# epam/ai-dial-rag

Hardware: AMD Instinct MI355X
Metric: retrieval_qps_10Mx384 (higher is better)
Workload: dtype f32 (int8 MFMA filter with exact integer dot products and a rigorous error margin, every candidate the margin cannot exclude re-scored in f64 with the reference formula)

## Files before the change

ai-dial-rag_amd/csrc/vec_index.hip:

```cpp
#include <algorithm>
#include <cmath>
#include <cstdarg>
#include <cstdio>
#include <cstdlib>
#include <cstring>
#include <mutex>
#include <new>
#include <type_traits>
#include <vector>

#include "common.h"
#include "vec_kernels.h"
#include "vec_kernels_f16.h"
#include "vec_kernels_q16.h"
#include "vec_kernels_h16.h"
#include "vec_kernels_sieve.h"
#include "vec_kernels_i8.h"
#include "vec_kernels_exact.h"

namespace mir {

static thread_local char g_err[512] = "";

void set_error(const char *fmt, ...) {
// ... 835 lines not shown
            sa.chunk_ids = ix->d_chunk; sa.doc_ids = ix->d_doc; sa.row_offset = ix->row_offset;
            sa.out_doc = o_doc; sa.out_chunk = o_chunk; sa.out_row = o_row; sa.out_dist = o_dist; sa.out_count = o_count;
            sa.out_flags = o_flags; sa.nflag = sb.nflag; sa.flagged = sb.flagged; sa.stats = ix->d_stats; sa.qt = sb.qt;
            rc = sieve(0, (uint32_t)kSampleWgs * pl.sample_tpw, kSampleWgs, nullptr, nullptr, nullptr, true);
            if (rc != MIR_OK) return rc;
            if (use_i8) {
                SieveSampleArgs ta;
                ta.part = reinterpret_cast<const float *>(sb.part_sample); ta.nwg = kSampleWgs; ta.qpw = qpw; ta.k = k; ta.nq = nq;
                ta.q0 = q0; ta.d = d; ta.metric = metric; ta.docs = ix->d_orig; ta.doc_sq = ix->d_docsq;
                ta.q = dq; ta.q_sq = sb.q_sq; ta.q_norm = sb.q_norm; ta.gthr = reinterpret_cast<unsigned long long *>(gt);
                sieve_sample_threshold_kernel<<<dim3(nq), dim3(256), 0, stream>>>(ta);
            } else {
                sample_threshold_kernel<<<dim3(nq), dim3(256), 0, stream>>>(reinterpret_cast<const float *>(sb.part_sample), kSampleWgs, qpw,
                                                                            k, nq, reinterpret_cast<unsigned long long *>(gt));
            }
            MIR_HIP(hipGetLastError());
            rc = begin_profile();
            if (rc != MIR_OK) return rc;
            for (int phase = pl.tiles_first ? 0 : 1; phase < 2 && rc == MIR_OK; ++phase) {
                const size_t region = use_i8 ? (size_t)kI8Region : (size_t)kSieveRegion;
                uint64_t *cand = sb.sv_cand + (size_t)phase * nwg * region;
                float *cv = sb.sv_candv + (size_t)phase * nwg * region;
                uint32_t *cc = sb.sv_ccount + (size_t)phase * nwg * (use_i8 ? 8 : 1);
                rc = phase == 0 ? sieve(0, pl.tiles_first, nwg, cand, cv, cc, false)
                                : sieve(pl.tiles_first, ix->n_tiles - pl.tiles_first, nwg, cand, cv, cc, false);
                if (rc != MIR_OK) break;
                if (phase == 1 && ev0) {
                    MIR_HIP(hipEventRecord(ev1, stream));
                    std::lock_guard<std::mutex> lk(ix->mu);
                    ix->prof_events.emplace_back(ev0, ev1);
                    ev1 = nullptr;
                }
                ca.cand = cand; ca.candv = cv; ca.ccount = cc;
                if (use_i8) sieve_scatter_i8_kernel<<<dim3(nwg * 8), dim3(256), 0, stream>>>(ca);
                else sieve_scatter_kernel<<<dim3(nwg * kSieveScatterSplit), dim3(256), 0, stream>>>(ca);
                sa.mode = phase;
                MIR_HIP(hipFuncSetAttribute(reinterpret_cast<const void *>(sieve_select_kernel), hipFuncAttributeMaxDynamicSharedMemorySize,
                                            (int)sieve_select_lds_bytes()));
                sieve_select_kernel<<<dim3(nq), dim3(kSieveSelectThreads), sieve_select_lds_bytes(), stream>>>(sa);
                MIR_HIP(hipGetLastError());
            }
            if (rc != MIR_OK) return rc;
            continue;
        }
        rc = begin_profile();
        if (rc != MIR_OK) return rc;
        if (qpw == 32) {
            rc = with_kind(metric, [&](auto kind) { return launch_scan<kind()>(ix, qs, nq, klist, nwg, pg, stream); });
        } else if (ix->native16) {
            const uint4 *qs16 = sb.qsplit + (size_t)g * (kQ16Queries / 16) * (ix->ksteps / 2) * 64;
            const float *qsc = sb.qscale + (size_t)g * qpw;
            rc = with_kind(metric, [&](auto kind) { return launch_scan_h16<kind()>(ix, qs16, qsc, nq, klist, nwg, pg, sb.gthr + (size_t)g * 128, stream); });
        } else if (ix->layout16) {
            const double *qn = sb.q_norm + (size_t)g * qpw;
            rc = with_kind(metric, [&](auto kind) { return launch_scan_q16<kind()>(ix, qs, qn, nq, klist, nwg, pg, stream); });
        } else {
            rc = with_kind(metric, [&](auto kind) { return launch_scan_f16<kind()>(ix, qs, nq, klist, nwg, pg, stream); });
        }
        if (ev1) {
            (void)hipEventRecord(ev1, stream);
            std::lock_guard<std::mutex> lk(ix->mu);
            ix->prof_events.emplace_back(ev0, ev1);
        }
        if (rc != MIR_OK) return rc;
    }
    if (pl.sieve) {
// ... 8 lines not shown
    fa.q = dq; fa.q_sq = sb.q_sq; fa.q_norm = sb.q_norm;
    fa.chunk_ids = ix->d_chunk; fa.doc_ids = ix->d_doc; fa.row_offset = ix->row_offset;
    fa.out_doc = o_doc; fa.out_chunk = o_chunk; fa.out_row = o_row; fa.out_dist = o_dist;
    fa.out_count = o_count; fa.out_flags = o_flags; fa.nflag = sb.nflag; fa.flagged = sb.flagged; fa.qt = sb.qt;
    finalize_kernel<<<dim3(b), dim3(256), 0, stream>>>(fa);
    MIR_HIP(hipGetLastError());
    exact_pass();
    MIR_HIP(hipGetLastError());
    return MIR_OK;
}

static int32_t plan(const mir_index *ix, int b, int k, SearchPlan *pl) {
    {
        const int64_t per_wg = (int64_t)b * std::min(k, kExactRound) * 16;
        const int64_t by_mem = std::max<int64_t>(64, ((int64_t)256 << 20) / std::max<int64_t>(per_wg, 1));
        pl->exact_grid = (int)std::max<int64_t>(1, std::min<int64_t>(std::min<int64_t>(ix->num_cus, by_mem), (ix->n + kXbRows - 1) / kXbRows));
    }
    pl->klist = std::min(k + (ix->native16 ? kH16ListMargin : kListMargin), kMaxList);
    auto exact_only = [&]() {
        pl->exact_only = true;
        pl->ngroups = 0;
        pl->qpw = 32;
        pl->nwg = 1;
        return MIR_OK;
    };
    if (ix->hi_only || ix->wide16 || (ix->native16 && sieve_sized(ix))) {
        if (k > kSieveMaxK) return exact_only();
        pl->sieve = true;
        pl->qpw = (ix->layout16 && b > kQ16Queries) ? kSieveMaxQueriesPerLaunch : kQ16Queries;
        pl->ngroups = (b + pl->qpw - 1) / pl->qpw;
        pl->nwg = (int)std::min<int64_t>(std::min(ix->num_cus, 1024), (int64_t)ix->n_tiles);
        pl->klist = std::min(k, kMaxList);
        const bool two = (int64_t)ix->n_tiles >= (int64_t)kSieveTwoLaunchTiles * pl->nwg;
        pl->tiles_first = two ? std::max<uint32_t>(ix->n_tiles / kSieveFirstDiv, std::min<uint32_t>(ix->n_tiles / 4, kSieveFirstMinTiles)) : 0;
        pl->tiles_first &= ~1u;
        pl->sample_tpw = std::max<uint32_t>(1, std::min<uint32_t>(kSampleTilesPerWg, ix->n_tiles / (4u * kSampleWgs)));
        return MIR_OK;
    }
    const bool wide64 = wide64_split(ix);
    const bool lists_fit = k + (ix->native16 ? kH16ListMargin : kListMargin) <= kMaxList;
    if (!lists_fit && ix->n > (int64_t)kMaxList) return exact_only();
    if (wide64 && f16_lds_bytes(pl->klist) <= 160 * 1024) {
        pl->qpw = kF16Queries;
        pl->ngroups = (b + pl->qpw - 1) / pl->qpw;
        const int64_t want16 = (int64_t)ix->n_tiles;
        pl->nwg = (int)std::max<int64_t>(1, std::min<int64_t>(std::min(ix->num_cus, 1024), want16));
        return MIR_OK;
    }
    if ((ix->layout16 || ix->native16) && pl->klist > kQ16MaxList) return exact_only();
    if (ix->layout16 || ix->native16) {
        pl->qpw = kQ16Queries;
        pl->ngroups = (b + pl->qpw - 1) / pl->qpw;
        pl->nwg = (int)std::max<int64_t>(1, std::min<int64_t>(std::min(ix->num_cus, 1024), (int64_t)ix->n_tiles));
        return MIR_OK;
    }
    pl->qpw = 32;
    pl->ngroups = (b + pl->qpw - 1) / pl->qpw;
    const int64_t want = (int64_t)ix->n_tiles;
    pl->nwg = (int)std::max<int64_t>(1, std::min<int64_t>(std::min(ix->num_cus, 1024), want));
    return MIR_OK;
}

}


struct ConcatItem {
    const void *src;
    int64_t dst_unit;
    int32_t n_units;
// ... 320 lines not shown
    std::vector<std::pair<hipEvent_t, hipEvent_t>> ev;
    {
        std::lock_guard<std::mutex> lk(idx->mu);
        ev.swap(idx->prof_events);
    }
    double ms = 0.0;
    for (auto &pr : ev) {
        float t = 0.f;
        hipError_t e = hipEventSynchronize(pr.second);
        if (e == hipSuccess) e = hipEventElapsedTime(&t, pr.first, pr.second);
        {
            std::lock_guard<std::mutex> lk(idx->mu);
            idx->prof_free.push_back(pr.first);
            idx->prof_free.push_back(pr.second);
        }
        if (e != hipSuccess) {
            set_error("profile read failed: %s", hipGetErrorString(e));
            return MIR_ERR_HIP;
        }
        ms += t;
    }
    std::lock_guard<std::mutex> lk(idx->mu);
    idx->prof_launches += (int64_t)ev.size();
    idx->prof_ms += ms;
    if (launches) *launches = idx->prof_launches;
    if (total_ms) *total_ms = idx->prof_ms;
    if (reset) {
        idx->prof_launches = 0;
        idx->prof_ms = 0.0;
    }
    return MIR_OK;
}

int32_t mir_index_scan_stats(mir_index *idx, int32_t reset, int64_t *out8) {
    MIR_REQUIRE(idx != nullptr && out8 != nullptr, "NULL argument");
    int32_t rc = use_device(idx->device, nullptr);
    if (rc != MIR_OK) return rc;
    MIR_HIP(hipDeviceSynchronize());
    MIR_HIP(hipMemcpy(out8, idx->d_stats, 64, hipMemcpyDeviceToHost));
    if (reset) MIR_HIP(hipMemset(idx->d_stats, 0, 64));
    out8[6] = idx->i8 ? 1 : 0;
    return MIR_OK;
}

int32_t mir_index_search_device(mir_index *idx, const double *queries_device, int32_t b, int32_t k,
                                int32_t metric, int32_t *out_doc, int64_t *out_chunk, int64_t *out_row,
                                double *out_dist, int32_t *out_count, int32_t *out_flags, void *stream_) {
    int32_t rc = check_search_args(idx, queries_device, b, k, metric, out_count);
    if (rc != MIR_OK) return rc;
    if (b == 0) return MIR_OK;
    hipStream_t stream = static_cast<hipStream_t>(stream_);
    rc = use_device(idx->device, nullptr);
    if (rc != MIR_OK) return rc;
    SearchPlan pl;
    rc = plan(idx, b, k, &pl);
    if (rc != MIR_OK) return rc;
    SearchBuffers sb;
    const size_t i8_rows = (idx->i8 && pl.sieve) ? (size_t)idx->n_stages * 64 : 0;
    const size_t need = carve(sb, nullptr, b, k, idx->d, std::max(idx->ksteps, idx->ks16), pl, false, i8_rows);
    Workspace *w = nullptr;
    rc = acquire_ws(idx, stream, need, &w);
    if (rc != MIR_OK) return rc;
    carve(sb, static_cast<char *>(w->buf), b, k, idx->d, std::max(idx->ksteps, idx->ks16), pl, false, i8_rows);
    rc = enqueue_search(idx, queries_device, b, k, metric, sb, pl, out_doc, out_chunk, out_row,
                        out_dist, out_count, out_flags, stream);
    release_ws(idx, w, stream, true);
    return rc;
}

int32_t mir_index_search(mir_index *idx, const double *queries_host, int32_t b, int32_t k, int32_t metric,
                         int32_t *out_doc, int64_t *out_chunk, int64_t *out_row, double *out_dist,
                         int32_t *out_count, int32_t *out_flags) {
    int32_t rc = check_search_args(idx, queries_host, b, k, metric, out_count);
    if (rc != MIR_OK) return rc;
// ... 185 lines not shown
```

ai-dial-rag_amd/csrc/vec_kernels_i8.h:

```cpp
#pragma once
#include "vec_kernels_sieve.h"

#ifndef I8_ABL
#define I8_ABL 0
#endif

namespace mir {

typedef int __attribute__((ext_vector_type(4))) i32x4;

constexpr int kI8StatWords = 8;
constexpr int kI8MaxK = 16;
static_assert(kI8MaxK <= kSieveSampleMaxK, "the exact sample threshold evaluates k rows in one round");
constexpr int kI8Region = 32768;
constexpr int kI8WavePart = kI8Region / 8;
__device__ __forceinline__ void i8_margin_ab(float qn, float eq, const float *__restrict__ stats, float &A, float &B) {
    i8_margin_ab_decl(qn, eq, stats, A, B);
}
__device__ __forceinline__ float i8_margin_tile(bool l2, float A, float B, float e_t, float s_t, float sq) {
    const float m = fmaf(e_t, A, B) + 2.0f * s_t * sq;
    return l2 ? 2.0f * m : m;
}

__global__ __launch_bounds__(256) void i8_tile_scale_kernel(const float *__restrict__ src, int64_t n, int d, float4 *__restrict__ tparam) {
// ... 404 lines not shown
        }
    }
    if (have_prev) {
#pragma unroll
        for (int u = 0; u < QT; ++u) filter(u, p0[u], p1[u], pax, pt, ptp);
    }
    if (SAMPLE) {
        uint32_t *part_row = reinterpret_cast<uint32_t *>(part_sample + (size_t)gridDim.x * QPL * 2);
#pragma unroll
        for (int u = 0; u < QT; ++u) {
            const float o = __shfl_xor(best[u], 16, 64);
            const uint32_t orow = (uint32_t)__shfl_xor((int)brow[u], 16, 64);
            const bool other = o > best[u];
            const float b2 = other ? o : best[u];
            const size_t at = ((size_t)blockIdx.x * QPL + qloc[u]) * 2 + (jg >> 1);
            if (lane_live[u] && (jg == 0 || jg == 2)) {
                part_sample[at] = b2;
                part_row[at] = other ? orow : brow[u];
            }
        }
        return;
    }
    if (lane == 0) {
        ccount[(size_t)blockIdx.x * NW + wave8] = wcount;
        if (stat && wcount) atomicAdd(stat, (unsigned long long)wcount);
    }
}

__global__ __launch_bounds__(256) void sieve_scatter_i8_kernel(SieveScatterArgs a) {
    __shared__ uint32_t s_cnt[256], s_base[256];
    const int tid = threadIdx.x;
    const int part = blockIdx.x;
    uint32_t cnt = a.ccount[part];
    s_cnt[tid] = 0;
    __syncthreads();
    if (cnt > (uint32_t)kI8WavePart) {
        for (int i = tid; i < a.nq; i += 256) a.l.over[a.q0 + i] = 1;
        cnt = kI8WavePart;
    }
    const uint64_t *region = a.cand + (size_t)part * kI8WavePart;
    const float *regionv = a.candv + (size_t)part * kI8WavePart;
    for (uint32_t e = tid; e < cnt; e += 256) atomicAdd(&s_cnt[(int)(region[e] >> 32) & 255], 1u);
    __syncthreads();
    {
        const uint32_t c = s_cnt[tid];
        s_base[tid] = c ? atomicAdd(&a.l.count[(size_t)(a.q0 + tid) * kSieveCountStride], c) : 0u;
        s_cnt[tid] = 0;
    }
    __syncthreads();
    for (uint32_t e = tid; e < cnt; e += 256) {
        const uint64_t key = region[e];
        const int ql = (int)(key >> 32) & 255, qi = a.q0 + ql;
        const uint32_t slot = s_base[ql] + atomicAdd(&s_cnt[ql], 1u);
        if (slot < (uint32_t)kSieveQueryCap) {
            a.l.row[(size_t)qi * kSieveQueryCap + slot] = (uint32_t)key;
            a.l.rv[(size_t)qi * kSieveQueryCap + slot] = regionv[e];
        } else {
            a.l.over[qi] = 1;
        }
    }
}

}
```

ai-dial-rag_amd/csrc/vec_kernels_sieve.h:

```cpp
#pragma once
#include "vec_kernels_q16.h"
#include "vec_kernels_h16.h"

#ifndef SIEVE_ABL
#define SIEVE_ABL 0
#endif
#ifndef SIEVE_MAX3
#define SIEVE_MAX3 1
#endif
#ifndef SIEVE_SELECT_ABL
#define SIEVE_SELECT_ABL 0
#endif
#ifndef SIEVE_PREFETCH
#define SIEVE_PREFETCH 2
#endif

namespace mir {

constexpr int kSieveStages = 6;
#ifndef MIR_SIEVE_REGION
#define MIR_SIEVE_REGION 8192
#endif
constexpr int kSieveRegion = MIR_SIEVE_REGION;
constexpr int kSieveQueryCap = 16384;
constexpr int kSieveSelectCap = 4096;
constexpr int kSieveMaxK = 64;
constexpr int kSieveCountStride = 32;

constexpr int kSieveAuxStride = kTileRows + 8;
__host__ __device__ constexpr size_t sieve_lds_bytes(int ks32) { return (size_t)kSieveStages * (ks32 * 2 * 1024 + kSieveAuxStride * 4) + 64; }

template <int KS32, int KIND, bool SAMPLE, int QT, bool PTMT>
__global__ __launch_bounds__(512, 2) void sieve_q16_kernel(const uint4 *__restrict__ docs, const float *__restrict__ aux,
                                                           const uint4 *__restrict__ qsplit, const double *__restrict__ q_norm,
                                                           const double *__restrict__ q_sq, const double *__restrict__ q_err,
                                                           const float *__restrict__ max_norm,
                                                           uint32_t n_rows, uint32_t tile0, uint32_t n_tiles, int nq, int nan_guard,
                                                           const uint64_t *__restrict__ gthr, uint64_t *__restrict__ cand,
                                                           float *__restrict__ candv, uint32_t *__restrict__ ccount,
                                                           float *__restrict__ part_sample, unsigned long long *__restrict__ stat,
                                                           uint32_t tile_u4,
                                                           const float *__restrict__ tile_max) {
    static_assert(QT == 1 || QT == 2, "query tiles per wave");
    constexpr int NS = kSieveStages;
// ... 469 lines not shown
        if (active) {
            p0 = c0; p1 = c1; pt = t; have_prev = true;
#pragma unroll
            for (int i = 0; i < 8; ++i) pax[i] = cax[i];
        }
    }
    if (have_prev) filter(p0, p1, pax, pt);
    if (SAMPLE) {
        const float o = __shfl_xor(best, 16, 64);
        const float b2 = fmaxf(best, o);
        if (lane_live && (jg == 0 || jg == 2)) part_sample[((size_t)blockIdx.x * kQ16Queries + qloc) * 2 + (jg >> 1)] = b2;
        return;
    }
    __syncthreads();
    if (tid == 0) {
        ccount[blockIdx.x] = *s_count;
        if (stat && *s_count) atomicAdd(stat, (unsigned long long)*s_count);
    }
}

struct SieveLists {
    float *rv;
    uint32_t *row;
    uint32_t *count;
    uint32_t *over;
};

struct SieveScatterArgs {
    const uint64_t *cand;
    const float *candv;
    const uint32_t *ccount;
    int q0, nq;
    SieveLists l;
};

constexpr int kSieveScatterSplit = 2;
__global__ __launch_bounds__(256) void sieve_scatter_kernel(SieveScatterArgs a) {
    const int tid = threadIdx.x;
    const int reg = blockIdx.x / kSieveScatterSplit, part = blockIdx.x % kSieveScatterSplit;
    uint32_t cnt = a.ccount[reg];
    if (cnt > (uint32_t)kSieveRegion) {
        if (part == 0)
            for (int i = tid; i < a.nq; i += 256) a.l.over[a.q0 + i] = 1;
        cnt = kSieveRegion;
    }
    const uint64_t *region = a.cand + (size_t)reg * kSieveRegion;
    const float *regionv = a.candv + (size_t)reg * kSieveRegion;
    for (uint32_t e = part * 256 + tid; e < cnt; e += 256 * kSieveScatterSplit) {
        const uint64_t key = region[e];
        const float v = regionv[e];
        const int qi = a.q0 + (int)(key >> 32);
        const uint32_t slot = atomicAdd(&a.l.count[(size_t)qi * kSieveCountStride], 1u);
        if (slot < (uint32_t)kSieveQueryCap) {
            a.l.row[(size_t)qi * kSieveQueryCap + slot] = (uint32_t)key;
            a.l.rv[(size_t)qi * kSieveQueryCap + slot] = v;
        } else {
            a.l.over[qi] = 1;
        }
    }
}

__device__ __forceinline__ uint32_t sieve_wave_max_u32(uint32_t x) {
#define MIR_DPP_MAX(CTRL)                                                                              \
    {                                                                                                  \
        const uint32_t o = (uint32_t)__builtin_amdgcn_update_dpp(0, (int)x, CTRL, 0xf, 0xf, false);    \
        x = x > o ? x : o;                                                                             \
// ... 130 lines not shown
    B = (stats[0] * eq + 3.0e-5f * stats[0] * qn) * (1.0f + 1e-5f) * MIR_MARGIN_SCALE;
}
struct SieveSelectArgs {
    SieveLists l;
    int q0, nq, k, metric, mode;
    int d, nan_guard;
    float rel_err;
    float extra_slop;
    const double *q_err;
    const float *i8_qscale;
    const float4 *i8_tparam;
    const float *docs;
    const _Float16 *docs16;
    const float *doc_sq;
    const float *dnorm;
    const double *q, *q_sq, *q_norm;
    const float *max_norm;
    unsigned long long *gthr;
    const int64_t *chunk_ids;
    const int32_t *doc_ids;
    int64_t row_offset;
    int32_t *out_doc;
    int64_t *out_chunk;
    int64_t *out_row;
    double *out_dist;
    int32_t *out_count;
    int32_t *out_flags;
    int32_t *nflag;
    int32_t *flagged;
    unsigned long long *stats;
    double *qt;
};

__host__ __device__ constexpr size_t sieve_select_lds_bytes() {
    return (size_t)kSieveQueryCap * 4 + 16 + (size_t)kSieveSelectCap * 18 + 16 * 64 * 4;
}
constexpr int kSieveSelectThreads = 1024;
__global__ __launch_bounds__(kSieveSelectThreads) void sieve_select_kernel(SieveSelectArgs a) {
    extern __shared__ __attribute__((aligned(16))) unsigned char sel_lds[];
    constexpr size_t kOffD = (size_t)kSieveQueryCap * 4 + 16;
    float *s_v = reinterpret_cast<float *>(sel_lds);
    double *s_d = reinterpret_cast<double *>(sel_lds + kOffD);
    float *s_x = reinterpret_cast<float *>(sel_lds + kOffD + (size_t)kSieveSelectCap * 8);
    uint32_t *s_row = reinterpret_cast<uint32_t *>(sel_lds + kOffD + (size_t)kSieveSelectCap * 12);
    uint16_t *s_fin = reinterpret_cast<uint16_t *>(sel_lds + kOffD + (size_t)kSieveSelectCap * 16);
    uint32_t *part = reinterpret_cast<uint32_t *>(sel_lds + kOffD + (size_t)kSieveSelectCap * 18);
    __shared__ int s_ns, s_f, s_f1, s_slot, s_have, s_nn;
    __shared__ float s_kv;
    constexpr int NT = kSieveSelectThreads;
    const int tid = threadIdx.x, lane = tid & 63, wave = tid >> 6;
    const int qi = a.q0 + blockIdx.x;
    const uint32_t total = a.l.count[(size_t)qi * kSieveCountStride];
    const int n = (int)(total < (uint32_t)kSieveQueryCap ? total : (uint32_t)kSieveQueryCap);
    const uint32_t *lr = a.l.row + (size_t)qi * kSieveQueryCap;
    const float *lv = a.l.rv + (size_t)qi * kSieveQueryCap;
    const bool over = a.l.over[qi] != 0;
    if (tid == 0) { s_ns = 0; s_f = 0; s_f1 = 0; s_have = 0; s_nn = 0; }
    __syncthreads();
    auto to_exact_pass = [&]() {
        if (a.mode != 1) return;
        if (tid == 0) {
            atomicAdd(a.stats + 3, 1ull);
            s_slot = atomicAdd(a.nflag, 1);
            a.flagged[s_slot] = qi;
            if (a.out_flags) a.out_flags[qi] = MIR_FLAG_EXACT_PASS;
            if (a.out_count) a.out_count[qi] = 0;
        }
        __syncthreads();
        exact_publish_query(a.qt, s_slot, a.q + (size_t)qi * a.d, a.d, a.metric, a.q_norm[qi], tid, NT);
    };
    if (over) {
        to_exact_pass();
        return;
    }
    auto kth_largest = [&](const float *vals, int m) -> float {
        __syncthreads();
        if (m <= NT) sieve_wave_topk<1>(vals, m, a.k, tid, NT, part + wave * 64);
        else if (m <= 2 * NT) sieve_wave_topk<2>(vals, m, a.k, tid, NT, part + wave * 64);
        else if (m <= 4 * NT) sieve_wave_topk<4>(vals, m, a.k, tid, NT, part + wave * 64);
        else sieve_wave_topk<kSieveQueryCap / kSieveSelectThreads>(vals, m, a.k, tid, NT, part + wave * 64);
        __syncthreads();
        if (wave == 0) {
            const int nw = m <= NT ? (m + 63) / 64 : NT / 64;
            uint32_t r[16];
#pragma unroll
            for (int j = 0; j < 16; ++j) {
                const int i = j * 64 + lane;
                r[j] = i < nw * a.k ? part[(i / a.k) * 64 + i % a.k] : 0u;
            }
            uint32_t wm = 0;
            for (int t = 0; t < a.k; ++t) wm = sieve_extract_max<16>(r, lane);
            if (lane == 0) s_kv = unorderable(wm);
        }
        __syncthreads();
        return s_kv;
    };
    const float qn = (float)a.q_norm[qi] * (1.0f + 1e-6f);
    const bool l2 = !(a.metric == MIR_METRIC_INNER_PRODUCT || a.metric == MIR_METRIC_COSINE_SIM);
    const float mg = a.q_err ? hihi_margin(a.metric == MIR_METRIC_COSINE_SIM, l2, qn, (float)a.q_err[qi] * (1.0f + 1e-6f), a.max_norm) +
                                   a.extra_slop * qn * (a.metric == MIR_METRIC_COSINE_SIM ? 1.0f : a.max_norm[0]) * (l2 ? 2.0f : 1.0f)
                             : a.rel_err * qn * (a.metric == MIR_METRIC_COSINE_SIM ? 1.0f : a.max_norm[0]) * (l2 ? 2.0f : 1.0f);
    const bool i8 = a.i8_qscale != nullptr;
    const bool per_row = i8 || (a.q_err != nullptr && a.dnorm != nullptr && a.metric != MIR_METRIC_COSINE_SIM);
    const float cq = (per_row && !i8) ? hihi_coeff(l2, qn, (float)a.q_err[qi] * (1.0f + 1e-6f), a.max_norm) : 0.f;
    float i8A = 0.f, i8B = 0.f;
    const float i8sq = i8 ? a.i8_qscale[qi] : 0.f;
    if (i8) {
        const float eq = (float)a.q_err[qi] * (1.0f + 1e-6f);
        if (qn < __builtin_inff() && eq < __builtin_inff()) i8_margin_ab_decl(qn, eq, a.max_norm, i8A, i8B);
        else i8A = i8B = __builtin_inff();
    }
    auto margin_of = [&](uint32_t row) {
        if (i8) {
            const float4 tp = a.i8_tparam[row / kTileRows];
            const float m = fmaf(tp.y, i8A, i8B) + 2.0f * tp.x * i8sq;
            return l2 ? 2.0f * m : a.metric == MIR_METRIC_COSINE_SIM ? m * a.max_norm[6] : m;
        }
        return per_row ? a.dnorm[row] * cq : mg;
    };
    const float eps_m = per_row ? 0.f : 1e-6f * mg;
    float guard = __builtin_inff();
    if (a.nan_guard) {
        const float qs = (float)a.q_sq[qi];
        guard = qs - 1e-5f * fabsf(qs);
    }
    for (int e0 = 0; e0 < n; e0 += NT) {
        const int e = e0 + tid;
        bool safe = false;
        if (e < n) {
            const float v = lv[e];
            const float m = margin_of(lr[e]);
            safe = v + m < guard && v > -__builtin_inff();
            s_v[e] = safe ? v - m : -__builtin_inff();
        }
        const unsigned long long bal = __ballot(safe);
        if (bal && lane == __builtin_ctzll(bal)) atomicAdd(&s_ns, __popcll(bal));
    }
    __syncthreads();
    const int ns = s_ns;
    const bool have = ns >= a.k;
    const float kv = have ? kth_largest(s_v, n) : 0.f;
    const float cut = have ? kv - 1e-5f * fabsf(kv) - eps_m : -__builtin_inff();
    auto compact = [&](int cls, int *counter) {
        for (int e0 = 0; e0 < n; e0 += NT) {
            const int e = e0 + tid;
            bool fin = false;
            if (e < n) {
                const float lb = s_v[e];
                const bool c1 = !have || !(lb > -__builtin_inff()) || !(lb < kv);
                if (a.mode == 0) fin = cls == 1 && lb > -__builtin_inff() && !(lb < kv);
                else if (cls == 1) fin = c1;
                else if (!c1) fin = !(lb + 2.0f * margin_of(lr[e]) * (1.0f + 1e-6f) < cut);
            }
            const unsigned long long bal = __ballot(fin);
            int base = 0;
            if (bal && lane == __builtin_ctzll(bal)) base = atomicAdd(counter, __popcll(bal));
            base = __shfl(base, bal ? __builtin_ctzll(bal) : 0, 64);
            const int slot = base + __popcll(bal & ((1ull << lane) - 1ull));
            if (fin && slot < kSieveSelectCap) { s_fin[slot] = (uint16_t)e; s_row[slot] = lr[e]; }
        }
        __syncthreads();
    };
    const double *qv = a.q + (size_t)qi * a.d;
    const double q_sq = a.q_sq[qi], q_norm = a.q_norm[qi];
    constexpr int GW = 16, GPW = 64 / GW;
    const int sub = lane / GW, lg = lane % GW;
    const bool vec4 = (a.d & 3) == 0;
    auto evaluate = [&](int lo, int hi) {
        for (int i0 = lo + wave * GPW; i0 < hi; i0 += (NT / 64) * GPW) {
            const int i = i0 + sub;
            const bool live = i < hi;
            const uint32_t row = s_row[live ? i : i0];
            double rv, dist;
            if (vec4) {
                dist = a.docs16 ? sieve_metric_g16<_Float16>(a.docs16 + (size_t)row * a.d, qv, a.d, a.metric, a.doc_sq[row], q_sq, q_norm, lg, &rv)
                                : sieve_metric_g16<float>(a.docs + (size_t)row * a.d, qv, a.d, a.metric, a.doc_sq[row], q_sq, q_norm, lg, &rv);
            } else {
                dist = a.docs16 ? exact_metric_wave<_Float16, GW, 8>(a.docs16 + (size_t)row * a.d, qv, a.d, a.metric, a.doc_sq[row], q_sq, q_norm, lg, &rv)
                                : exact_metric_wave<float, GW, 8>(a.docs + (size_t)row * a.d, qv, a.d, a.metric, a.doc_sq[row], q_sq, q_norm, lg, &rv);
            }
            if (live && lg == 0) {
                s_d[i] = dist;
                s_x[i] = dist == dist ? (float)rv : -__builtin_inff();
            }
        }
        __syncthreads();
    };
    auto count_numeric = [&](int m) {
        for (int i0 = 0; i0 < m; i0 += NT) {
            const int i = i0 + tid;
            const bool num = i < m && s_x[i] > -__builtin_inff();
            const unsigned long long bal = __ballot(num);
            if (bal && lane == __builtin_ctzll(bal)) atomicAdd(&s_nn, __popcll(bal));
        }
        __syncthreads();
    };
    if (a.mode == 0) {
        if (have) {
            float thr = kv - 4e-6f * fabsf(kv) - eps_m;
            compact(1, &s_f);
            const int f1 = s_f;
            if (f1 <= kSieveSelectCap) {
                evaluate(0, f1);
                count_numeric(f1);
                if (s_nn >= a.k) {
                    const float rk = kth_largest(s_x, f1);
                    const float need = rk - 4e-6f * fabsf(rk) - eps_m;
                    thr = need > thr ? need : thr;
                }
            }
            if (tid == 0) {
                const unsigned long long key = (unsigned long long)orderable(thr) << 32;
                if (thr == thr && key > a.gthr[blockIdx.x]) a.gthr[blockIdx.x] = key;
            }
        }
        if (tid == 0) atomicAdd(a.stats + 4, (unsigned long long)n);
        return;
    }
    compact(1, &s_f);
    const int f1 = s_f;
    if (tid == 0) s_f1 = f1;
    compact(2, &s_f);
    int f = s_f;
    if (f > kSieveSelectCap) {
        to_exact_pass();
        return;
    }
#if SIEVE_SELECT_ABL == 1
    return;
#endif
    const bool two_rounds = f - f1 > 128;
    evaluate(0, two_rounds ? f1 : f);
#if SIEVE_SELECT_ABL == 2
    return;
#endif
    if (two_rounds) {
        count_numeric(f1);
        if (s_nn >= a.k) {
            const float rk = kth_largest(s_x, f1);
            const float need = rk - 4e-6f * fabsf(rk) - eps_m;
            if (tid == 0) s_f = f1;
            __syncthreads();
            for (int i0 = f1; i0 < f; i0 += NT) {
                const int i = i0 + tid;
                uint16_t e = 0;
                uint32_t er = 0;
                bool keep = false;
                if (i < f) {
                    e = s_fin[i];
                    er = s_row[i];
                    keep = !(s_v[e] + 2.0f * margin_of(er) * (1.0f + 1e-6f) < need);
                }
                __syncthreads();
                const unsigned long long bal = __ballot(keep);
                int base = 0;
                if (bal && lane == __builtin_ctzll(bal)) base = atomicAdd(&s_f, __popcll(bal));
                base = __shfl(base, bal ? __builtin_ctzll(bal) : 0, 64);
                const int slot = base + __popcll(bal & ((1ull << lane) - 1ull));
                if (keep) { s_fin[slot] = e; s_row[slot] = er; }
                __syncthreads();
            }
            f = s_f;
        }
        evaluate(f1, f);
    }
    bool pre = false;
    if (f > 256) {
        for (int i0 = 0; i0 < f; i0 += NT) {
            const int i = i0 + tid;
            if (i < f) {
                const double dd = s_d[i];
                s_x[i] = dd == dd ? -(float)dd : -__builtin_inff();
            }
        }
        if (tid == 0) s_nn = 0;
        __syncthreads();
        for (int i0 = 0; i0 < f; i0 += NT) {
            const int i = i0 + tid;
            const bool num = i < f && s_x[i] > -__builtin_inff();
            const unsigned long long bal = __ballot(num);
            if (bal && lane == __builtin_ctzll(bal)) atomicAdd(&s_nn, __popcll(bal));
        }
        __syncthreads();
        pre = s_nn >= a.k;
    }
    const float kx = pre ? kth_largest(s_x, f) : -__builtin_inff();
    const int kout = a.k < f ? a.k : f;
    for (int i = tid; i < f; i += NT) {
        if (pre && s_x[i] < kx) continue;
        const double dd = s_d[i];
        const uint32_t rr = s_row[i];
        int rank = 0;
        for (int c = 0; c < f; ++c) {
            if (pre && s_x[c] < kx) continue;
            rank += dist_before(s_d[c], s_row[c], dd, rr) ? 1 : 0;
        }
        if (rank < a.k) {
            const size_t o = (size_t)qi * a.k + rank;
            if (a.out_row) a.out_row[o] = a.row_offset + (int64_t)rr;
            if (a.out_dist) a.out_dist[o] = dd;
            if (a.out_doc) a.out_doc[o] = a.doc_ids ? a.doc_ids[rr] : 0;
            if (a.out_chunk) a.out_chunk[o] = a.chunk_ids ? a.chunk_ids[rr] : (int64_t)rr;
        }
    }
    if (tid == 0) {
        atomicAdd(a.stats + 5, (unsigned long long)f);
        atomicAdd(a.stats + 2, 1ull);
        if (a.out_count) a.out_count[qi] = kout;
        if (a.out_flags) a.out_flags[qi] = 0;
    }
}

constexpr int kSieveSampleMaxK = 16;
struct SieveSampleArgs {
    const float *part;
    int nwg, qpw, k, nq, q0, d, metric;
    const float *docs, *doc_sq;
    const double *q, *q_sq, *q_norm;
    unsigned long long *gthr;
};
__global__ __launch_bounds__(256) void sieve_sample_threshold_kernel(SieveSampleArgs a) {
    constexpr int kMaxVals = 2 * 256;
    __shared__ unsigned long long keys[kMaxVals];
    __shared__ float s_x[kSieveSampleMaxK];
    const int tid = threadIdx.x, lane = tid & 63, wave = tid >> 6;
    const int q = blockIdx.x;
    if (q >= a.nq || a.k > kSieveSampleMaxK) return;
    const uint32_t *prow = reinterpret_cast<const uint32_t *>(a.part + (size_t)a.nwg * a.qpw * 2);
    const int n = 2 * a.nwg;
    for (int e = tid; e < kMaxVals; e += 256) {
        unsigned long long key = 0;
        if (e < n) {
            const size_t at = ((size_t)(e >> 1) * a.qpw + q) * 2 + (e & 1);
            const float v = a.part[at];
            if (v > -__builtin_inff()) key = ((unsigned long long)orderable(v) << 32) | prow[at];
        }
        keys[e] = key;
    }
    for (int size = 2; size <= kMaxVals; size <<= 1)
        for (int stride = size >> 1; stride > 0; stride >>= 1) {
            __syncthreads();
            const int lo = 2 * tid - (tid & (stride - 1)), hi = lo + stride;
            const bool desc = (lo & size) == 0;
            const unsigned long long x = keys[lo], y = keys[hi];
            if ((x < y) == desc) {
                keys[lo] = y;
                keys[hi] = x;
            }
        }
    __syncthreads();
    if (keys[a.k - 1] == 0) return;
    const int qi = a.q0 + q;
    const double *qv = a.q + (size_t)qi * a.d;
    const double q_sq = a.q_sq[qi], q_norm = a.q_norm[qi];
    const int sub = lane >> 4, lg = lane & 15;
    for (int i0 = wave * 4; i0 < a.k; i0 += 16) {
        const int i = i0 + sub;
        const bool live = i < a.k;
        const uint32_t row = (uint32_t)keys[live ? i : i0];
        double rv, dist;
        if ((a.d & 3) == 0)
            dist = sieve_metric_g16<float>(a.docs + (size_t)row * a.d, qv, a.d, a.metric, a.doc_sq[row], q_sq, q_norm, lg, &rv);
        else
            dist = exact_metric_wave<float, 16, 8>(a.docs + (size_t)row * a.d, qv, a.d, a.metric, a.doc_sq[row], q_sq, q_norm, lg, &rv);
        if (live && lg == 0) s_x[i] = dist == dist ? (float)rv : -__builtin_inff();
    }
    __syncthreads();
    if (tid == 0) {
        float thr = key_value(keys[a.k - 1]);
        int nn = 0;
        for (int i = 0; i < a.k; ++i) nn += s_x[i] > -__builtin_inff() ? 1 : 0;
        if (nn == a.k) {
            float rk = s_x[0];
            for (int i = 1; i < a.k; ++i) rk = fminf(rk, s_x[i]);
            const float need = rk - 4e-6f * fabsf(rk);
            thr = need > thr ? need : thr;
        }
        a.gthr[q] = (unsigned long long)orderable(thr) << 32;
    }
}

}
// ... 1 lines not shown
```

Baseline: 255,500.

## Streamline sieve select: single-pass two-class compaction, wave-parallel ranking, cheaper sample top-k

The select kernel now compacts both candidate classes in one pass into opposite ends of the shared buffer, where it used to make two passes. It caches per-entry margins in LDS, prefetches the first list entries before the barrier, and sizes the partial-max merge to the real count. Small finalist sets are ranked by 16-lane groups with shuffle reductions instead of one serial loop per thread. The sample threshold kernel replaces a 512-element bitonic sort with register-based wave top-k extraction. The change also adds env-driven plan sweep knobs and timestamp probes behind compile flags, and raises the select kernel's LDS use, which may affect occupancy.

```diff
diff --git a/ai-dial-rag_amd/csrc/vec_index.hip b/ai-dial-rag_amd/csrc/vec_index.hip
--- a/ai-dial-rag_amd/csrc/vec_index.hip
+++ b/ai-dial-rag_amd/csrc/vec_index.hip
@@ -891,6 +891,9 @@
                     ev1 = nullptr;
                 }
                 ca.cand = cand; ca.candv = cv; ca.ccount = cc;
+#ifdef MIR_SIEVE_PLAN_SWEEP
+                ca.max_part = ix->d_stats + 6;
+#endif
                 if (use_i8) sieve_scatter_i8_kernel<<<dim3(nwg * 8), dim3(256), 0, stream>>>(ca);
                 else sieve_scatter_kernel<<<dim3(nwg * kSieveScatterSplit), dim3(256), 0, stream>>>(ca);
                 sa.mode = phase;
@@ -965,9 +968,16 @@
         pl->nwg = (int)std::min<int64_t>(std::min(ix->num_cus, 1024), (int64_t)ix->n_tiles);
         pl->klist = std::min(k, kMaxList);
         const bool two = (int64_t)ix->n_tiles >= (int64_t)kSieveTwoLaunchTiles * pl->nwg;
-        pl->tiles_first = two ? std::max<uint32_t>(ix->n_tiles / kSieveFirstDiv, std::min<uint32_t>(ix->n_tiles / 4, kSieveFirstMinTiles)) : 0;
+        uint32_t first_div = kSieveFirstDiv, first_min = kSieveFirstMinTiles, sample_tpw = kSampleTilesPerWg;
+#ifdef MIR_SIEVE_PLAN_SWEEP
+        auto sweep = [](const char *name, uint32_t dflt) { const char *v = getenv(name); return v && *v ? (uint32_t)atoi(v) : dflt; };
+        first_div = std::max(1u, sweep("MIR_SWEEP_FIRST_DIV", first_div));
+        first_min = sweep("MIR_SWEEP_FIRST_MIN", first_min);
+        sample_tpw = std::max(1u, sweep("MIR_SWEEP_SAMPLE_TPW", sample_tpw));
+#endif
+        pl->tiles_first = two ? std::max<uint32_t>(ix->n_tiles / first_div, std::min<uint32_t>(ix->n_tiles / 4, first_min)) : 0;
         pl->tiles_first &= ~1u;
-        pl->sample_tpw = std::max<uint32_t>(1, std::min<uint32_t>(kSampleTilesPerWg, ix->n_tiles / (4u * kSampleWgs)));
+        pl->sample_tpw = std::max<uint32_t>(1, std::min<uint32_t>(sample_tpw, ix->n_tiles / (4u * kSampleWgs)));
         return MIR_OK;
     }
     const bool wide64 = wide64_split(ix);
@@ -1354,6 +1364,16 @@
     return MIR_OK;
 }
 
+#ifdef SIEVE_SELECT_STAMPS
+extern "C" int32_t mir_debug_select_stamps(unsigned long long *out32) {
+    MIR_HIP(hipDeviceSynchronize());
+    MIR_HIP(hipMemcpyFromSymbol(out32, HIP_SYMBOL(mir::g_sieve_select_stamps), 32 * sizeof(unsigned long long)));
+    unsigned long long zero[32] = {};
+    MIR_HIP(hipMemcpyToSymbol(HIP_SYMBOL(mir::g_sieve_select_stamps), zero, sizeof(zero)));
+    return MIR_OK;
+}
+#endif
+
 int32_t mir_index_scan_stats(mir_index *idx, int32_t reset, int64_t *out8) {
     MIR_REQUIRE(idx != nullptr && out8 != nullptr, "NULL argument");
     int32_t rc = use_device(idx->device, nullptr);
@@ -1361,7 +1381,9 @@
     MIR_HIP(hipDeviceSynchronize());
     MIR_HIP(hipMemcpy(out8, idx->d_stats, 64, hipMemcpyDeviceToHost));
     if (reset) MIR_HIP(hipMemset(idx->d_stats, 0, 64));
+#ifndef MIR_SIEVE_PLAN_SWEEP
     out8[6] = idx->i8 ? 1 : 0;
+#endif
     return MIR_OK;
 }
 
diff --git a/ai-dial-rag_amd/csrc/vec_kernels_i8.h b/ai-dial-rag_amd/csrc/vec_kernels_i8.h
--- a/ai-dial-rag_amd/csrc/vec_kernels_i8.h
+++ b/ai-dial-rag_amd/csrc/vec_kernels_i8.h
@@ -460,6 +460,9 @@
     const int tid = threadIdx.x;
     const int part = blockIdx.x;
     uint32_t cnt = a.ccount[part];
+#ifdef MIR_SIEVE_PLAN_SWEEP
+    if (tid == 0) atomicMax(a.max_part, (unsigned long long)cnt);
+#endif
     s_cnt[tid] = 0;
     __syncthreads();
     if (cnt > (uint32_t)kI8WavePart) {
diff --git a/ai-dial-rag_amd/csrc/vec_kernels_sieve.h b/ai-dial-rag_amd/csrc/vec_kernels_sieve.h
--- a/ai-dial-rag_amd/csrc/vec_kernels_sieve.h
+++ b/ai-dial-rag_amd/csrc/vec_kernels_sieve.h
@@ -1,4 +1,5 @@
 #pragma once
+#include <type_traits>
 #include "vec_kernels_q16.h"
 #include "vec_kernels_h16.h"
 
@@ -10,6 +11,19 @@
 #endif
 #ifndef SIEVE_SELECT_ABL
 #define SIEVE_SELECT_ABL 0
+#endif
+#ifdef SIEVE_SELECT_STAMPS
+#define SIEVE_STAMP(seg)                                                                                  \
+    {                                                                                                     \
+        __builtin_amdgcn_sched_barrier(0);                                                                \
+        unsigned long long t_;                                                                            \
+        asm volatile("s_memtime %0\n\ts_waitcnt lgkmcnt(0)" : "=s"(t_)::"memory");                        \
+        __builtin_amdgcn_sched_barrier(0);                                                                \
+        if (blockIdx.x == 0 && threadIdx.x == 0) atomicAdd(&g_sieve_select_stamps[a.mode & 1][seg], t_ - stamp_prev); \
+        stamp_prev = t_;                                                                                  \
+    }
+#else
+#define SIEVE_STAMP(seg)
 #endif
 #ifndef SIEVE_PREFETCH
 #define SIEVE_PREFETCH 2
@@ -545,6 +559,9 @@
     const uint32_t *ccount;
     int q0, nq;
     SieveLists l;
+#ifdef MIR_SIEVE_PLAN_SWEEP
+    unsigned long long *max_part;
+#endif
 };
 
 constexpr int kSieveScatterSplit = 2;
@@ -741,10 +758,16 @@
     double *qt;
 };
 
+constexpr int kSieveSelectMarginLds = 4096;
 __host__ __device__ constexpr size_t sieve_select_lds_bytes() {
-    return (size_t)kSieveQueryCap * 4 + 16 + (size_t)kSieveSelectCap * 18 + 16 * 64 * 4;
-}
+    return (size_t)kSieveQueryCap * 4 + 16 + (size_t)kSieveSelectCap * 18 + 16 * 64 * 4 + (size_t)kSieveSelectMarginLds * 4;
+}
+static_assert(sieve_select_lds_bytes() + 256 <= 160 * 1024, "the select kernel's LDS");
 constexpr int kSieveSelectThreads = 1024;
+constexpr int kSieveRankDirect = 256;
+#ifdef SIEVE_SELECT_STAMPS
+__device__ unsigned long long g_sieve_select_stamps[2][16];
+#endif
 __global__ __launch_bounds__(kSieveSelectThreads) void sieve_select_kernel(SieveSelectArgs a) {
     extern __shared__ __attribute__((aligned(16))) unsigned char sel_lds[];
     constexpr size_t kOffD = (size_t)kSieveQueryCap * 4 + 16;
@@ -754,7 +777,8 @@
     uint32_t *s_row = reinterpret_cast<uint32_t *>(sel_lds + kOffD + (size_t)kSieveSelectCap * 12);
     uint16_t *s_fin = reinterpret_cast<uint16_t *>(sel_lds + kOffD + (size_t)kSieveSelectCap * 16);
     uint32_t *part = reinterpret_cast<uint32_t *>(sel_lds + kOffD + (size_t)kSieveSelectCap * 18);
-    __shared__ int s_ns, s_f, s_f1, s_slot, s_have, s_nn;
+    float *s_m = reinterpret_cast<float *>(part + 16 * 64);
+    __shared__ int s_ns, s_f, s_f2, s_slot, s_nn;
     __shared__ float s_kv;
     constexpr int NT = kSieveSelectThreads;
     const int tid = threadIdx.x, lane = tid & 63, wave = tid >> 6;
@@ -764,8 +788,16 @@
     const uint32_t *lr = a.l.row + (size_t)qi * kSieveQueryCap;
     const float *lv = a.l.rv + (size_t)qi * kSieveQueryCap;
     const bool over = a.l.over[qi] != 0;
-    if (tid == 0) { s_ns = 0; s_f = 0; s_f1 = 0; s_have = 0; s_nn = 0; }
+    static_assert(kSieveQueryCap >= kSieveSelectThreads, "the list's first entries are read before its count is known");
+    const float v_first = lv[tid];
+    const uint32_t row_first = lr[tid];
+    if (tid == 0) { s_ns = 0; s_f = 0; s_f2 = 0; s_nn = 0; }
     __syncthreads();
+#ifdef SIEVE_SELECT_STAMPS
+    unsigned long long stamp_prev;
+    asm volatile("s_memtime %0\n\ts_waitcnt lgkmcnt(0)" : "=s"(stamp_prev)::"memory");
+    if (blockIdx.x == 0 && tid == 0) atomicAdd(&g_sieve_select_stamps[a.mode & 1][15], 1ull);
+#endif
     auto to_exact_pass = [&]() {
         if (a.mode != 1) return;
         if (tid == 0) {
@@ -791,14 +823,25 @@
         __syncthreads();
         if (wave == 0) {
             const int nw = m <= NT ? (m + 63) / 64 : NT / 64;
-            uint32_t r[16];
-#pragma unroll
-            for (int j = 0; j < 16; ++j) {
-                const int i = j * 64 + lane;
-                r[j] = i < nw * a.k ? part[(i / a.k) * 64 + i % a.k] : 0u;
-            }
-            uint32_t wm = 0;
-            for (int t = 0; t < a.k; ++t) wm = sieve_extract_max<16>(r, lane);
+            const int nk = nw * a.k;
+            auto merge = [&](auto rc) {
+                constexpr int R = decltype(rc)::value;
+                uint32_t r[R];
+#pragma unroll
+                for (int j = 0; j < R; ++j) {
+                    const int i = j * 64 + lane;
+                    r[j] = i < nk ? part[(i / a.k) * 64 + i % a.k] : 0u;
+                }
+                uint32_t wm = 0;
+                for (int t = 0; t < a.k; ++t) wm = sieve_extract_max<R>(r, lane);
+                return wm;
+            };
+            uint32_t wm;
+            if (nw == 1) wm = part[a.k - 1];
+            else if (nk <= 64) wm = merge(std::integral_constant<int, 1>());
+            else if (nk <= 128) wm = merge(std::integral_constant<int, 2>());
+            else if (nk <= 256) wm = merge(std::integral_constant<int, 4>());
+            else wm = merge(std::integral_constant<int, 16>());
             if (lane == 0) s_kv = unorderable(wm);
         }
         __syncthreads();
@@ -833,40 +876,53 @@
         const float qs = (float)a.q_sq[qi];
         guard = qs - 1e-5f * fabsf(qs);
     }
+    const bool m_lds = n <= kSieveSelectMarginLds;
+    auto margin_at = [&](int e, uint32_t row) { return m_lds ? s_m[e] : margin_of(row); };
     for (int e0 = 0; e0 < n; e0 += NT) {
         const int e = e0 + tid;
         bool safe = false;
         if (e < n) {
-            const float v = lv[e];
-            const float m = margin_of(lr[e]);
+            const float v = e0 == 0 ? v_first : lv[e];
+            const float m = margin_of(e0 == 0 ? row_first : lr[e]);
             safe = v + m < guard && v > -__builtin_inff();
             s_v[e] = safe ? v - m : -__builtin_inff();
+            if (m_lds) s_m[e] = m;
         }
         const unsigned long long bal = __ballot(safe);
         if (bal && lane == __builtin_ctzll(bal)) atomicAdd(&s_ns, __popcll(bal));
     }
     __syncthreads();
+    SIEVE_STAMP(0)
     const int ns = s_ns;
     const bool have = ns >= a.k;
     const float kv = have ? kth_largest(s_v, n) : 0.f;
+    SIEVE_STAMP(1)
     const float cut = have ? kv - 1e-5f * fabsf(kv) - eps_m : -__builtin_inff();
-    auto compact = [&](int cls, int *counter) {
+    int split = kSieveSelectCap;
+    auto at = [&](int i) { return i < split ? i : kSieveSelectCap - 1 - (i - split); };
+    auto compact = [&](bool both) {
         for (int e0 = 0; e0 < n; e0 += NT) {
             const int e = e0 + tid;
-            bool fin = false;
+            bool fin1 = false, fin2 = false;
+            uint32_t row = 0;
             if (e < n) {
                 const float lb = s_v[e];
                 const bool c1 = !have || !(lb > -__builtin_inff()) || !(lb < kv);
-                if (a.mode == 0) fin = cls == 1 && lb > -__builtin_inff() && !(lb < kv);
-                else if (cls == 1) fin = c1;
-                else if (!c1) fin = !(lb + 2.0f * margin_of(lr[e]) * (1.0f + 1e-6f) < cut);
-            }
-            const unsigned long long bal = __ballot(fin);
-            int base = 0;
-            if (bal && lane == __builtin_ctzll(bal)) base = atomicAdd(counter, __popcll(bal));
-            base = __shfl(base, bal ? __builtin_ctzll(bal) : 0, 64);
-            const int slot = base + __popcll(bal & ((1ull << lane) - 1ull));
-            if (fin && slot < kSieveSelectCap) { s_fin[slot] = (uint16_t)e; s_row[slot] = lr[e]; }
+                if (!both) fin1 = lb > -__builtin_inff() && !(lb < kv);
+                else if (c1) fin1 = true;
+                else fin2 = !(lb + 2.0f * margin_at(e, m_lds ? 0u : lr[e]) * (1.0f + 1e-6f) < cut);
+                if (fin1 || fin2) row = lr[e];
+            }
+            const unsigned long long bal1 = __ballot(fin1), bal2 = __ballot(fin2);
+            const unsigned long long lt = (1ull << lane) - 1ull;
+            int base1 = 0, base2 = 0;
+            if (bal1 && lane == __builtin_ctzll(bal1)) base1 = atomicAdd(&s_f, __popcll(bal1));
+            if (bal2 && lane == __builtin_ctzll(bal2)) base2 = atomicAdd(&s_f2, __popcll(bal2));
+            base1 = __shfl(base1, bal1 ? __builtin_ctzll(bal1) : 0, 64);
+            base2 = __shfl(base2, bal2 ? __builtin_ctzll(bal2) : 0, 64);
+            const int slot1 = base1 + __popcll(bal1 & lt), slot2 = base2 + __popcll(bal2 & lt);
+            if (fin1 && slot1 < kSieveSelectCap) { s_fin[slot1] = (uint16_t)e; s_row[slot1] = row; }
+            if (fin2 && slot2 < kSieveSelectCap) { s_fin[kSieveSelectCap - 1 - slot2] = (uint16_t)e; s_row[kSieveSelectCap - 1 - slot2] = row; }
         }
         __syncthreads();
     };
@@ -879,7 +935,7 @@
         for (int i0 = lo + wave * GPW; i0 < hi; i0 += (NT / 64) * GPW) {
             const int i = i0 + sub;
             const bool live = i < hi;
-            const uint32_t row = s_row[live ? i : i0];
+            const uint32_t row = s_row[at(live ? i : i0)];
             double rv, dist;
             if (vec4) {
                 dist = a.docs16 ? sieve_metric_g16<_Float16>(a.docs16 + (size_t)row * a.d, qv, a.d, a.metric, a.doc_sq[row], q_sq, q_norm, lg, &rv)
@@ -907,16 +963,19 @@
     if (a.mode == 0) {
         if (have) {
             float thr = kv - 4e-6f * fabsf(kv) - eps_m;
-            compact(1, &s_f);
+            compact(false);
+            SIEVE_STAMP(2)
             const int f1 = s_f;
             if (f1 <= kSieveSelectCap) {
                 evaluate(0, f1);
+                SIEVE_STAMP(3)
                 count_numeric(f1);
                 if (s_nn >= a.k) {
                     const float rk = kth_largest(s_x, f1);
                     const float need = rk - 4e-6f * fabsf(rk) - eps_m;
                     thr = need > thr ? need : thr;
                 }
+                SIEVE_STAMP(4)
             }
             if (tid == 0) {
                 const unsigned long long key = (unsigned long long)orderable(thr) << 32;
@@ -924,13 +983,15 @@
             }
         }
         if (tid == 0) atomicAdd(a.stats + 4, (unsigned long long)n);
+#ifdef MIR_SIEVE_PLAN_SWEEP
+        if (tid == 0) atomicMax(a.stats + 7, (unsigned long long)total);
+#endif
         return;
     }
-    compact(1, &s_f);
+    compact(true);
+    SIEVE_STAMP(2)
     const int f1 = s_f;
-    if (tid == 0) s_f1 = f1;
-    compact(2, &s_f);
-    int f = s_f;
+    int f = f1 + s_f2;
     if (f > kSieveSelectCap) {
         to_exact_pass();
         return;
@@ -938,8 +999,10 @@
 #if SIEVE_SELECT_ABL == 1
     return;
 #endif
+    split = f1;
     const bool two_rounds = f - f1 > 128;
     evaluate(0, two_rounds ? f1 : f);
+    SIEVE_STAMP(3)
 #if SIEVE_SELECT_ABL == 2
     return;
 #endif
@@ -948,7 +1011,7 @@
         if (s_nn >= a.k) {
             const float rk = kth_largest(s_x, f1);
             const float need = rk - 4e-6f * fabsf(rk) - eps_m;
-            if (tid == 0) s_f = f1;
+            if (tid == 0) s_f2 = 0;
             __syncthreads();
             for (int i0 = f1; i0 < f; i0 += NT) {
                 const int i = i0 + tid;
@@ -956,25 +1019,26 @@
                 uint32_t er = 0;
                 bool keep = false;
                 if (i < f) {
-                    e = s_fin[i];
-                    er = s_row[i];
-                    keep = !(s_v[e] + 2.0f * margin_of(er) * (1.0f + 1e-6f) < need);
+                    e = s_fin[at(i)];
+                    er = s_row[at(i)];
+                    keep = !(s_v[e] + 2.0f * margin_at(e, er) * (1.0f + 1e-6f) < need);
                 }
                 __syncthreads();
                 const unsigned long long bal = __ballot(keep);
                 int base = 0;
-                if (bal && lane == __builtin_ctzll(bal)) base = atomicAdd(&s_f, __popcll(bal));
+                if (bal && lane == __builtin_ctzll(bal)) base = atomicAdd(&s_f2, __popcll(bal));
                 base = __shfl(base, bal ? __builtin_ctzll(bal) : 0, 64);
-                const int slot = base + __popcll(bal & ((1ull << lane) - 1ull));
-                if (keep) { s_fin[slot] = e; s_row[slot] = er; }
+                const int slot = f1 + base + __popcll(bal & ((1ull << lane) - 1ull));
+                if (keep) { s_fin[at(slot)] = e; s_row[at(slot)] = er; }
                 __syncthreads();
             }
-            f = s_f;
+            f = f1 + s_f2;
         }
         evaluate(f1, f);
     }
+    SIEVE_STAMP(4)
     bool pre = false;
-    if (f > 256) {
+    if (f > kSieveRankDirect) {
         for (int i0 = 0; i0 < f; i0 += NT) {
             const int i = i0 + tid;
             if (i < f) {
@@ -995,23 +1059,49 @@
     }
     const float kx = pre ? kth_largest(s_x, f) : -__builtin_inff();
     const int kout = a.k < f ? a.k : f;
-    for (int i = tid; i < f; i += NT) {
-        if (pre && s_x[i] < kx) continue;
-        const double dd = s_d[i];
-        const uint32_t rr = s_row[i];
-        int rank = 0;
-        for (int c = 0; c < f; ++c) {
-            if (pre && s_x[c] < kx) continue;
-            rank += dist_before(s_d[c], s_row[c], dd, rr) ? 1 : 0;
-        }
-        if (rank < a.k) {
-            const size_t o = (size_t)qi * a.k + rank;
-            if (a.out_row) a.out_row[o] = a.row_offset + (int64_t)rr;
-            if (a.out_dist) a.out_dist[o] = dd;
-            if (a.out_doc) a.out_doc[o] = a.doc_ids ? a.doc_ids[rr] : 0;
-            if (a.out_chunk) a.out_chunk[o] = a.chunk_ids ? a.chunk_ids[rr] : (int64_t)rr;
-        }
-    }
+    auto put = [&](int rank, double dd, uint32_t rr) {
+        const size_t o = (size_t)qi * a.k + rank;
+        if (a.out_row) a.out_row[o] = a.row_offset + (int64_t)rr;
+        if (a.out_dist) a.out_dist[o] = dd;
+        if (a.out_doc) a.out_doc[o] = a.doc_ids ? a.doc_ids[rr] : 0;
+        if (a.out_chunk) a.out_chunk[o] = a.chunk_ids ? a.chunk_ids[rr] : (int64_t)rr;
+    };
+    if (f <= kSieveRankDirect) {
+        for (int i0 = wave * GPW; i0 < f; i0 += (NT / 64) * GPW) {
+            const int i = i0 + sub;
+            const bool live = i < f;
+            double dd = 0.0;
+            uint32_t rr = 0;
+            int rank = 0;
+            if (live) {
+                dd = s_d[i];
+                rr = s_row[at(i)];
+                for (int c = lg; c < f; c += GW) rank += dist_before(s_d[c], s_row[at(c)], dd, rr) ? 1 : 0;
+            }
+#pragma unroll
+            for (int off = GW / 2; off >= 1; off >>= 1) rank += __shfl_xor(rank, off, 64);
+            if (live && lg == 0 && rank < a.k) put(rank, dd, rr);
+        }
+    } else {
+        for (int i = tid; i < f; i += NT) {
+            if (pre && s_x[i] < kx) continue;
+            const double dd = s_d[i];
+            const uint32_t rr = s_row[at(i)];
+            int rank = 0;
+            for (int c = 0; c < f; ++c) {
+                if (pre && s_x[c] < kx) continue;
+                rank += dist_before(s_d[c], s_row[at(c)], dd, rr) ? 1 : 0;
+            }
+            if (rank < a.k) put(rank, dd, rr);
+        }
+    }
+#ifdef SIEVE_SELECT_STAMPS
+    __syncthreads();
+    SIEVE_STAMP(5)
+#endif
+#ifdef MIR_SIEVE_PLAN_SWEEP
+    if (tid == 0) atomicMax(a.stats + 7, (unsigned long long)total);
+#endif
     if (tid == 0) {
         atomicAdd(a.stats + 5, (unsigned long long)f);
         atomicAdd(a.stats + 2, 1ull);
@@ -1028,35 +1118,60 @@
     const double *q, *q_sq, *q_norm;
     unsigned long long *gthr;
 };
+template <int R>
+__device__ __forceinline__ unsigned long long sieve_extract_max64(unsigned long long (&r)[R], int lane) {
+    unsigned long long m = r[0];
+#pragma unroll
+    for (int j = 1; j < R; ++j) m = r[j] > m ? r[j] : m;
+    const uint32_t wh = sieve_wave_max_u32((uint32_t)(m >> 32));
+    const uint32_t wl = sieve_wave_max_u32((uint32_t)(m >> 32) == wh ? (uint32_t)m : 0u);
+    const unsigned long long wm = ((unsigned long long)wh << 32) | wl;
+    const unsigned long long bal = __ballot(m == wm);
+    if (wm != 0 && lane == __builtin_ctzll(bal)) {
+        bool done = false;
+#pragma unroll
+        for (int j = 0; j < R; ++j) {
+            const bool hit = !done && r[j] == wm;
+            r[j] = hit ? 0ull : r[j];
+            done = done || hit;
+        }
+    }
+    return wm;
+}
 __global__ __launch_bounds__(256) void sieve_sample_threshold_kernel(SieveSampleArgs a) {
     constexpr int kMaxVals = 2 * 256;
-    __shared__ unsigned long long keys[kMaxVals];
+    __shared__ unsigned long long s_part[4 * kSieveSampleMaxK];
+    __shared__ unsigned long long keys[kSieveSampleMaxK];
     __shared__ float s_x[kSieveSampleMaxK];
     const int tid = threadIdx.x, lane = tid & 63, wave = tid >> 6;
     const int q = blockIdx.x;
     if (q >= a.nq || a.k > kSieveSampleMaxK) return;
     const uint32_t *prow = reinterpret_cast<const uint32_t *>(a.part + (size_t)a.nwg * a.qpw * 2);
     const int n = 2 * a.nwg;
-    for (int e = tid; e < kMaxVals; e += 256) {
-        unsigned long long key = 0;
+    unsigned long long r[kMaxVals / 256];
+#pragma unroll
+    for (int j = 0; j < kMaxVals / 256; ++j) {
+        const int e = j * 256 + tid;
+        r[j] = 0;
         if (e < n) {
             const size_t at = ((size_t)(e >> 1) * a.qpw + q) * 2 + (e & 1);
             const float v = a.part[at];
-            if (v > -__builtin_inff()) key = ((unsigned long long)orderable(v) << 32) | prow[at];
-        }
-        keys[e] = key;
-    }
-    for (int size = 2; size <= kMaxVals; size <<= 1)
-        for (int stride = size >> 1; stride > 0; stride >>= 1) {
-            __syncthreads();
-            const int lo = 2 * tid - (tid & (stride - 1)), hi = lo + stride;
-            const bool desc = (lo & size) == 0;
-            const unsigned long long x = keys[lo], y = keys[hi];
-            if ((x < y) == desc) {
-                keys[lo] = y;
-                keys[hi] = x;
-            }
-        }
+            if (v > -__builtin_inff()) r[j] = ((unsigned long long)orderable(v) << 32) | prow[at];
+        }
+    }
+    for (int t = 0; t < a.k; ++t) {
+        const unsigned long long wm = sieve_extract_max64(r, lane);
+        if (lane == 0) s_part[wave * kSieveSampleMaxK + t] = wm;
+    }
+    __syncthreads();
+    if (wave == 0) {
+        unsigned long long r2[1];
+        r2[0] = lane < 4 * a.k ? s_part[(lane / a.k) * kSieveSampleMaxK + lane % a.k] : 0ull;
+        for (int t = 0; t < a.k; ++t) {
+            const unsigned long long wm = sieve_extract_max64(r2, lane);
+            if (lane == 0) keys[t] = wm;
+        }
+    }
     __syncthreads();
     if (keys[a.k - 1] == 0) return;
     const int qi = a.q0 + q;
```

New measurement: 260,500, median of 6. 1.02x the previous value.
